# castorini/howl

Measured on AMD Instinct MI355X. Metric: utterances/sec/node (res8 end-to-end training step, 1s@16kHz, 40-mel), higher is better.
Workload: dtype f32; 1 GPU; res8 training step (frontend+fwd+xent+bwd+AdamW), 512 x 1 s utterances per GPU, 12 labels -- BASELINE configs[2] per-GPU share: res8 GSC-12, 512 x 1 s per GPU (4096 over 8); global_batch=512, samples_per_utterance=16000, labels=12, parallelism=single, frontend=eval

## Files before the change

howl_amd/csrc/res8.hip:

```cpp
#include "howl_common.hip.h"
#include "../../include/howl_hip.h"

namespace {

struct HowlPtrs6 {
    float* p[6];
};
constexpr int MAX_WINDOWS = 64;
struct HowlWinRows {
    int lo[MAX_WINDOWS], hi[MAX_WINDOWS];
};
struct HowlBnBuffers {
    float* running_mean;
    float* running_var;
    long long* num_batches;
};
struct BnFold {
    const float* part;
    int nparts;
    double count;
    float* stats_out;
    HowlBnBuffers bn;
};

// ... 1558 lines not shown
                const unsigned bc = (4u * idx[u] + 2u * h) / (unsigned)P;
                const unsigned bb = bc / NMAP;
                cc[u][h] = bc - bb * NMAP;
                if (dx == nullptr) gb[h] = dpool[bb * CP + cc[u][h]] * invP;
            }
            g[u] = dx != nullptr ? reinterpret_cast<const float4*>(dx)[idx[u]] : make_float4(gb[0], gb[0], gb[1], gb[1]);
            sv[u] = reinterpret_cast<const float4*>(s)[idx[u]];
            kk[u] = dskip != nullptr ? reinterpret_cast<const float4*>(dskip)[idx[u]] : make_float4(0.0f, 0.0f, 0.0f, 0.0f);
        }
#pragma unroll
        for (int u = 0; u < 2; ++u) {
            float2 dsa, dza, dsb, dzb;
            finish(make_float2(g[u].x, g[u].y), make_float2(sv[u].x, sv[u].y), make_float2(kk[u].x, kk[u].y), cc[u][0], dsa, dza);
            finish(make_float2(g[u].z, g[u].w), make_float2(sv[u].z, sv[u].w), make_float2(kk[u].z, kk[u].w), cc[u][1], dsb, dzb);
            if (ok[u]) {
                if (ds_out != nullptr) reinterpret_cast<float4*>(ds_out)[idx[u]] = make_float4(dsa.x, dsa.y, dsb.x, dsb.y);
                reinterpret_cast<float4*>(dz_out)[idx[u]] = make_float4(dza.x, dza.y, dzb.x, dzb.y);
            }
        }
    }
    if ((n2 & 1u) && blockIdx.x == 0 && tid == 0) {
        const unsigned i = n2 - 1;
        const unsigned bc = (2u * i) / (unsigned)P;
        const unsigned bb = bc / NMAP, c = bc - bb * NMAP;
        float2 g;
        if (dx != nullptr) {
            g = reinterpret_cast<const float2*>(dx)[i];
        } else {
            const float v = dpool[bb * CP + c] * invP;
            g = make_float2(v, v);
        }
        const float2 sv = reinterpret_cast<const float2*>(s)[i];
        const float2 kk = dskip != nullptr ? reinterpret_cast<const float2*>(dskip)[i] : make_float2(0.0f, 0.0f);
        float2 ds, dz;
        finish(g, sv, kk, c, ds, dz);
        if (ds_out != nullptr) reinterpret_cast<float2*>(ds_out)[i] = ds;
        reinterpret_cast<float2*>(dz_out)[i] = dz;
    }
}


template <bool EXACT = false>
__device__ __forceinline__ void load_feat_tile(float* tin, const float* feat, long sb, long st, long sm, int b, int T,
                                               int M, int tid, int nthreads, int t_lo = 0, int t_hi = 0) {
    const int pitch = M + 4;
    const int n = (T + 2) * pitch;
    for (int i0 = tid; i0 < n; i0 += 8 * nthreads) {
        float v[8];
#pragma unroll
        for (int j = 0; j < 8; ++j) {
            const int i = i0 + j * nthreads;
            const int t = i / pitch - 1, m = i % pitch - 1;
            const bool ok = i < n && (EXACT ? t >= t_lo && t < t_hi : t >= 0 && t < T) && m >= 0 && m < M;
            v[j] = feat[b * sb + (ok ? t * st + m * sm : 0)];
        }
#pragma unroll
        for (int j = 0; j < 8; ++j) {
            const int i = i0 + j * nthreads;
            const int t = i / pitch - 1, m = i % pitch - 1;
            const bool ok = (EXACT ? t >= t_lo && t < t_hi : t >= 0 && t < T) && m >= 0 && m < M;
            if (i < n) tin[i] = ok ? v[j] : 0.0f;
        }
    }
}

constexpr int C0M_THREADS = 512;

template <int NS = 1, bool EXACT = false>
__global__ __launch_bounds__(C0M_THREADS) void conv0_fwd_mfma_kernel(const float* __restrict__ feat, long sb, long st,
                                                                    long sm, const float* __restrict__ w0,
                                                                    float* __restrict__ s0, unsigned short* __restrict__ mask0,
                                                                    int B, int T, int M, int H, int nconv, HowlPtrs6 cw,
                                                                    float* __restrict__ wp_fwd, float* __restrict__ wp_bwd,
                                                                    int nwin, int win_step, int win_last, int slices) {
    if ((int)blockIdx.x >= nconv) {
        const int e = ((int)blockIdx.x - nconv) * C0M_THREADS + (int)threadIdx.x;
        if (e < 2 * 6 * PACK_ELEMS) pack_weights_one(cw, wp_fwd, wp_bwd, (e / PACK_ELEMS) % 6, e / (6 * PACK_ELEMS), e % PACK_ELEMS);
        return;
    }
    HIP_DYNAMIC_SHARED(float, lds)
    float* tin = lds;
    const int tid = threadIdx.x, lane = tid & 63, wave = tid >> 6;
    const int pitch = M + 4;
    const int P = H * PW;
    const int g = lane >> 4, n = lane & 15;
    float bw[3][3];
#pragma unroll
    for (int ks = 0; ks < 3; ++ks)
#pragma unroll
        for (int nt = 0; nt < 3; ++nt) {
            const int tap = 4 * ks + g, c = 16 * nt + n;
            bw[ks][nt] = (tap < 9 && c < NMAP) ? w0[c * 9 + tap] : 0.0f;
        }
    int aoff[3];
#pragma unroll
    for (int ks = 0; ks < 3; ++ks) {
        const int tap = min(4 * ks + g, 8);
        aoff[ks] = (tap / 3) * pitch + tap % 3 + (n & 7) + (n >> 3) * 3 * pitch;
    }
    for (int i = tid; i < 3 * pitch + 16; i += C0M_THREADS) tin[(T + 2) * pitch + i] = 0.0f;
    for (int item = blockIdx.x; item < B * slices; item += nconv) {
        const int b = item / slices, sl = item - b * slices;
        const int ph0 = (sl * H) / slices, ph1 = ((sl + 1) * H) / slices;
        __syncthreads();
        const int clip = b / nwin, wi = b - clip * nwin;
        const int t0 = EXACT ? wi * win_step : min(wi * win_step, win_last);
        load_feat_tile<EXACT>(tin, feat + (long)clip * sb + (long)t0 * st, 0, st, sm, 0, T, M, tid, C0M_THREADS, -t0, win_last - t0);
        __syncthreads();
        constexpr int NJ = 5 * NS;
        for (int u = wave; u < NJ * ((ph1 - ph0 + 1) / 2); u += C0M_THREADS / 64) {
            const int pp = u / NJ, j8 = u - NJ * pp;
            const float* rowp = tin + 3 * (ph0 + 2 * pp) * pitch + 8 * j8;
            {
                f32x4 acc[3][3];
#pragma unroll
                for (int tl = 0; tl < 3; ++tl)
#pragma unroll
                    for (int nt = 0; nt < 3; ++nt) acc[tl][nt] = {0.0f, 0.0f, 0.0f, 0.0f};
#pragma unroll
                for (int tl = 0; tl < 3; ++tl)
#pragma unroll
                    for (int ks = 0; ks < 3; ++ks) {
                        const float a = rowp[aoff[ks] + tl * pitch];
#pragma unroll
                        for (int nt = 0; nt < 3; ++nt)
                            acc[tl][nt] = __builtin_amdgcn_mfma_f32_16x16x4f32(a, bw[ks][nt], acc[tl][nt], 0, 0, 0);
                    }
                const int pw = 2 * j8 + (g & 1), ph = ph0 + 2 * pp + (g >> 1);
#pragma unroll
                for (int nt = 0; nt < 3; ++nt) {
                    float sum = 0.0f;
                    unsigned bits = 0;
#pragma unroll
                    for (int tl = 0; tl < 3; ++tl)
#pragma unroll
                        for (int r = 0; r < 4; ++r) {
                            const int rb = max(__float_as_int(acc[tl][nt][r]), 0);
                            sum += __int_as_float(rb);
                            bits |= min((unsigned)rb, 1u) << (4 * tl + r);
                        }
                    const int c = 16 * nt + n;
                    if (ph < ph1 && c < NMAP) {
                        const int strip = NS > 1 ? pw / PW : 0;
                        const size_t o = (((size_t)b * NS + strip) * NMAP + c) * P + (size_t)ph * PW + (pw - strip * PW);
                        s0[o] = sum * (1.0f / 12.0f);
                        if (mask0 != nullptr) mask0[o] = (unsigned short)bits;
                    }
                }
            }
        }
    }
}

constexpr int C0G_WAVES = 15, C0G_THREADS = 64 * C0G_WAVES, C0G_CPW = NMAP / C0G_WAVES;
static_assert(C0G_CPW * C0G_WAVES == NMAP, "channels split evenly over the waves");

__device__ __forceinline__ void load_patch(float (&x)[5][6], const float* tin, int pitch, int ph, int pw) {
    const float* base = tin + 3 * ph * pitch + 4 * pw;
#pragma unroll
    for (int r = 0; r < 5; ++r) {
        const float4 a = *reinterpret_cast<const float4*>(base + r * pitch);
        const float2 c = *reinterpret_cast<const float2*>(base + r * pitch + 4);
        x[r][0] = a.x, x[r][1] = a.y, x[r][2] = a.z, x[r][3] = a.w, x[r][4] = c.x, x[r][5] = c.y;
    }
}

template <int NS = 1, bool EXACT = false>
__global__ __launch_bounds__(C0G_THREADS) void conv0_wgrad_valu_kernel(const float* __restrict__ feat, long sb, long st, long sm,
                                                                      const unsigned short* __restrict__ mask0,
                                                                      const float* __restrict__ ga, const float* __restrict__ gb,
                                                                      float* __restrict__ part, int B, int T, int M, int H,
                                                                      int slices, StripGeom sg, int t_total) {
    HIP_DYNAMIC_SHARED(float, lds)
    float* tin = lds;
    const int tid = threadIdx.x, lane = tid & 63;
    const int wave = __builtin_amdgcn_readfirstlane(tid >> 6);
    const int pitch = M + 4;
    const int P = H * PW;
    float acc[C0G_CPW][9];
#pragma unroll
    for (int j = 0; j < C0G_CPW; ++j)
#pragma unroll
        for (int t = 0; t < 9; ++t) acc[j][t] = 0.0f;
    const int nrs = EXACT ? sg.nr : 1;
    for (int item = blockIdx.x; item < B * nrs * NS * slices; item += gridDim.x) {
        const int vb = item / slices, sl = item - vb * slices;
        const int vq = NS > 1 ? vb / NS : vb, strip = NS > 1 ? vb - vq * NS : 0;
        const int b = EXACT ? vq / nrs : vq, rs = EXACT ? vq - b * nrs : 0;
        const int Pv = (EXACT && rs == nrs - 1) ? sg.hv_last * PW : P;
        const int cell0 = (sl * Pv) / slices, cell1 = ((sl + 1) * Pv) / slices;
        __syncthreads();
        if constexpr (EXACT)
            load_feat_tile<true>(tin, feat + (long)rs * T * st, sb, st, sm, b, T, M, tid, C0G_THREADS, -rs * T, t_total - rs * T);
        else
            load_feat_tile(tin, feat, sb, st, sm, b, T, M, tid, C0G_THREADS);
        __syncthreads();
        const float* gab = ga + ((size_t)vb * NMAP + C0G_CPW * wave) * P;
        const float* gbb = gb != nullptr ? gb + ((size_t)vb * NMAP + C0G_CPW * wave) * P : nullptr;
        const unsigned short* mb = mask0 + ((size_t)vb * NMAP + C0G_CPW * wave) * P;
        for (int cb = cell0; cb < cell1; cb += 64) {
            const int cell = cb + lane;
            const bool valid = cell < cell1;
            const unsigned cc = (unsigned)(valid ? cell : cell1 - 1);
            float gv[C0G_CPW];
            unsigned mv[C0G_CPW];
#pragma unroll
            for (int j = 0; j < C0G_CPW; ++j) {
                const unsigned o = (unsigned)(j * P) + cc;
                gv[j] = gab[o] + (gbb != nullptr ? gbb[o] : 0.0f);
                mv[j] = mb[o];
            }
            const int ph = (int)cc / PW, pw = (int)cc - ph * PW;
            float x[5][6];
            load_patch(x, tin, pitch, ph, pw + strip * PW);
#pragma unroll
            for (int j = 0; j < C0G_CPW; ++j) {
                const int gbits = valid ? __float_as_int(gv[j] * (1.0f / 12.0f)) : 0;
#pragma unroll
                for (int tl = 0; tl < 3; ++tl)
#pragma unroll
                    for (int fl = 0; fl < 4; ++fl) {
                        const int k = 4 * tl + fl;
                        const int sel = ((int)(mv[j] << (31 - k))) >> 31;
                        const float dy = __int_as_float(sel & gbits);
#pragma unroll
                        for (int tap = 0; tap < 9; ++tap) acc[j][tap] = fmaf(dy, x[tl + tap / 3][fl + tap % 3], acc[j][tap]);
                    }
            }
        }
    }
#pragma unroll
    for (int j = 0; j < C0G_CPW; ++j)
#pragma unroll
        for (int t = 0; t < 9; ++t) {
            const float v = wave_sum_rows(acc[j][t]);
            if (lane == 0) part[(size_t)blockIdx.x * NMAP * 9 + (C0G_CPW * wave + j) * 9 + t] = v;
        }
}

constexpr int HEAD_XC = 64;
constexpr int HEAD_THREADS = 768, HEAD_PARTS = 16;
__global__ __launch_bounds__(HEAD_THREADS) void head_fwd_kernel(const float* __restrict__ s6, const float* __restrict__ stats,
                                                       const float* __restrict__ wout, const float* __restrict__ bout,
                                                       float* __restrict__ pooled, float* __restrict__ logits, int B,
                                                       int P, int C, const long long* __restrict__ labels,
                                                       float* __restrict__ nll, float* __restrict__ dlogits,
                                                       float* __restrict__ dpool, float inv_batch,
                                                       const float* __restrict__ pool, int npg, int npg_used, BnFold fold,
                                                       int ns ) {
    __shared__ float lp[CP];
    __shared__ float ll[HEAD_XC], dl[HEAD_XC], lse_s;
    __shared__ float lst[2 * CP];
    __shared__ float lw[HEAD_XC * NMAP];
    __shared__ float lparts[HEAD_PARTS][CP];
    const int tid = threadIdx.x, lane = tid & 63, wave = tid >> 6;
    const bool w_in_lds = C <= HEAD_XC;
    if (w_in_lds)
        for (int i = tid; i < C * NMAP; i += HEAD_THREADS) lw[i] = wout[i];
    if (fold.part != nullptr) {
        const int c8 = lane >> 3;
        for (int w0 = wave; w0 < CP / 4; w0 += HEAD_THREADS / 64) {
            const int c = 4 * w0 + (c8 & 3);
            const double sm = fold_part_column(fold.part, part_stride(fold.nparts), fold.nparts, (c8 < 4 ? 0 : CP) + c, lane);
            const double q = __shfl_xor(sm, 32);
            if (c8 < 4 && (lane & 7) == 0) {
                const double mean = sm / fold.count;
                double var = q / fold.count - mean * mean;
                var = var < 0.0 ? 0.0 : var;
                const float fm = (c < NMAP) ? (float)mean : 0.0f;
                const float fr = (c < NMAP) ? (float)(1.0 / sqrt(var + (double)BN_EPS)) : 0.0f;
                lst[c] = fm;
                lst[CP + c] = fr;
                if (blockIdx.x == 0) {
                    fold.stats_out[c] = fm;
                    fold.stats_out[CP + c] = fr;
                    if (c < NMAP && fold.bn.running_mean != nullptr) {
                        const double unbiased = fold.count > 1.0 ? var * fold.count / (fold.count - 1.0) : var;
                        fold.bn.running_mean[c] = (1.0f - BN_MOMENTUM) * fold.bn.running_mean[c] + BN_MOMENTUM * (float)mean;
                        fold.bn.running_var[c] = (1.0f - BN_MOMENTUM) * fold.bn.running_var[c] + BN_MOMENTUM * (float)unbiased;
                    }
                    if (c == 0 && fold.bn.num_batches != nullptr) fold.bn.num_batches[0] += 1;
                }
            }
        }
    } else if (tid < 2 * CP) {
        lst[tid] = stats[tid];
    }
    __syncthreads();
    for (int b = blockIdx.x; b < B; b += gridDim.x) {
        __syncthreads();
        if (pool != nullptr) {
            const int nparts = ns * npg_used;
            const int pc = tid % CP, pk = tid / CP;
            float acc = 0.0f;
            for (int k0 = 0; k0 < nparts; k0 += HEAD_PARTS) {
                const int k = k0 + pk;
                if (k < nparts) {
                    const int sgi = k / npg_used, g = k - sgi * npg_used;
                    lparts[pk][pc] = pool[(((size_t)b * ns + sgi) * npg + g) * CP + pc];
                }
                __syncthreads();
                if (tid < CP) {
                    const int n = nparts - k0 < HEAD_PARTS ? nparts - k0 : HEAD_PARTS;
                    for (int j = 0; j < n; ++j) acc += lparts[j][tid];
                }
                __syncthreads();
            }
            if (tid < CP) {
                const float v = tid < NMAP ? (acc / (float)P - lst[tid]) * lst[CP + tid] : 0.0f;
                lp[tid] = v;
                pooled[(size_t)b * CP + tid] = v;
            }
        } else if (wave < 4)
        for (int c0 = wave; c0 < CP; c0 += 12) {
            float a8[3][8];
#pragma unroll
            for (int u = 0; u < 3; ++u) {
                const int c = c0 + 4 * u < NMAP ? c0 + 4 * u : NMAP - 1;
                const float* src = s6 + ((size_t)b * NMAP + c) * P;
#pragma unroll
                for (int j = 0; j < 8; ++j) a8[u][j] = src[min(lane + 64 * j, P - 1)];
            }
#pragma unroll
            for (int u = 0; u < 3; ++u) {
                const int c = c0 + 4 * u;
#pragma unroll
                for (int j = 0; j < 8; ++j) a8[u][j] = (lane + 64 * j < P) ? fabsf(a8[u][j]) : 0.0f;
                float acc = ((a8[u][0] + a8[u][1]) + (a8[u][2] + a8[u][3])) + ((a8[u][4] + a8[u][5]) + (a8[u][6] + a8[u][7]));
                acc = wave_sum(acc);
                const float v = c < NMAP ? (acc / (float)P - lst[c]) * lst[CP + c] : 0.0f;
                if (lane == 0 && c < CP) {
                    lp[c] = v;
                    pooled[(size_t)b * CP + c] = v;
                }
            }
        }
        __syncthreads();
        for (int k = tid; k < C; k += HEAD_THREADS) {
            float acc = bout[k];
            if (w_in_lds)
                for (int c = 0; c < NMAP; ++c) acc = fmaf(lw[k * NMAP + c], lp[c], acc);
            else
                for (int c = 0; c < NMAP; ++c) acc = fmaf(wout[k * NMAP + c], lp[c], acc);
            logits[(size_t)b * C + k] = acc;
            if (labels != nullptr) ll[k] = acc;
        }
        if (labels == nullptr) continue;
        __syncthreads();
        const int y = (int)labels[b];
        if (tid == 0) {
            float mx = ll[0];
            for (int k = 1; k < C; ++k) mx = fmaxf(mx, ll[k]);
            float se = 0.0f;
            for (int k = 0; k < C; ++k) se += expf(ll[k] - mx);
            const float lse = mx + logf(se);
            lse_s = lse;
            nll[b] = lse - ll[y];
        }
        __syncthreads();
        if (tid < C) {
            const float d = (expf(ll[tid] - lse_s) - (tid == y ? 1.0f : 0.0f)) * inv_batch;
            dl[tid] = d;
            dlogits[(size_t)b * C + tid] = d;
        }
        __syncthreads();
        if (tid < CP) {
            float acc = 0.0f;
            if (tid < NMAP)
                for (int k = 0; k < C; ++k) acc = fmaf(dl[k], lw[k * NMAP + tid], acc);
            dpool[(size_t)b * CP + tid] = acc;
        }
    }
}

__global__ __launch_bounds__(256) void head_fwd_windows_kernel(const float* __restrict__ s6, const float* __restrict__ stats,
                                                               const float* __restrict__ wout, const float* __restrict__ bout,
                                                               float* __restrict__ logits, int B, int nwin, int Hw,
                                                               HowlWinRows rows, float inv_count, int C, int ns) {
    __shared__ float lp[CP];
    const int tid = threadIdx.x, lane = tid & 63, wave = tid >> 6;
    const int Pw = Hw * PW;
    for (int b = blockIdx.x; b < B; b += gridDim.x) {
        __syncthreads();
        for (int c = wave; c < CP; c += 4) {
            float acc = 0.0f;
            if (c < NMAP) {
                for (int w = 0; w < nwin * ns; ++w) {
                    const float* src = s6 + ((size_t)(b * nwin * ns + w) * NMAP + c) * Pw;
                    for (int i = rows.lo[w / ns] * PW + lane; i < rows.hi[w / ns] * PW; i += 64) acc += fabsf(src[i]);
                }
// ... 142 lines not shown
    if ((threadIdx.x & 63) == 0) red[threadIdx.x >> 6] = acc;
    __syncthreads();
    if (threadIdx.x == 0) {
        double tot = 0.0;
        for (int w = 0; w < 16; ++w) tot += red[w];
        loss[0] = (float)(tot / (double)B);
    }
}

__global__ void adamw_kernel(float* __restrict__ p, const float* __restrict__ g, float* __restrict__ m,
                             float* __restrict__ v, size_t n, HowlAdamWCoef c) {
    for (size_t i = (size_t)blockIdx.x * blockDim.x + threadIdx.x; i < n; i += (size_t)gridDim.x * blockDim.x)
        howl_adamw_element(p, m, v, i, g[i], c);
}

}

namespace {

size_t conv0_tile_floats(int T, int M) { return (size_t)(T + 2) * (M + 4) + 3 * (M + 4) + 16; }
size_t conv_lds_bytes(int H, bool own_rows) {
    return (size_t)(3 * KSTEPS * 64 + tile_floats(H, own_rows) + 4 * CP + 12 * 2 * 16) * sizeof(float);
}
size_t wgrad_lds_bytes(int H) { return (size_t)(tile_floats_z(H) + tile_floats_x(H) + 6 * CP) * sizeof(float); }

struct Ws {
    float* wp_fwd;
    float* wp_bwd;
    float* part;
    float* part2;
    float* stats;
    float* m12;
    float* dpool;
    float* pool;
    float* bufa;
    float* bufb;
    float* dz;
    float* dz2;
    float* dsa;
    float* dsb;
    float* wpart;
    float* c0part;
};

size_t ws_layout(Ws* w, char* base, int B, int H, int G, int cus, size_t* fwd_eval_bytes) {
    size_t off = 0;
    auto take = [&](size_t floats) {
        float* p = base ? reinterpret_cast<float*>(base + off) : nullptr;
        off += ((floats * sizeof(float) + 255) / 256) * 256;
        return p;
    };
    const size_t act = (size_t)B * NMAP * H * PW;
    w->wp_fwd = take((size_t)6 * 3 * KSTEPS * 64);
    w->wp_bwd = take((size_t)6 * 3 * KSTEPS * 64);
    const int max_parts = G > cus ? G : cus;
    w->part = take((size_t)part_stride(max_parts) * 2 * CP);
    w->part2 = take((size_t)part_stride(max_parts) * 2 * CP);
    w->stats = take((size_t)6 * 2 * CP);
    w->m12 = take(2 * CP);
    w->dpool = take((size_t)B * CP);
    w->pool = take((size_t)B * 16 * CP);
    *fwd_eval_bytes = off;
    w->bufa = take(act);
    w->bufb = take(act);
    w->dz = take(act);
    w->dz2 = take(act);
    w->dsa = take(act);
    w->dsb = take(act);
    w->wpart = take((size_t)6 * G * CP * WNCOL);
    w->c0part = take((size_t)max_parts * NMAP * 9);
    return off;
}

int mel_strips(int M) { return M == 40 ? 1 : (M == 80 ? 2 : 0); }
int even_grid(int g, int strips) { return strips > 1 ? ((g & ~1) > 2 ? (g & ~1) : 2) : g; }
int launch_blocks(int nblk, int per_group) { return 8 * per_group * ((nblk + 7) / 8); }
int conv_slices(int nblk, int H, int budget) {
    const int ntiles = (H * PW + 15) / 16;
    for (int sl = 4; sl > 1; sl >>= 1)
        if (nblk * sl <= budget && 4 * sl <= ntiles) return sl;
    return 1;
}
void pair_slices(int nblk, int H, int cus, int* sd, int* sw) {
    const int ntiles = (H * PW + 15) / 16;
    const int opts[3][2] = {{4, 2}, {2, 2}, {2, 1}};
    *sd = *sw = 1;
    for (const auto& o : opts)
        if (nblk * (o[0] + o[1]) <= cus && 4 * o[0] <= ntiles) {
            *sd = o[0];
            *sw = o[1];
            return;
        }
}
int conv0_slices(int B, int cus) {
    const int sl = cus / (B > 0 ? B : 1);
    return sl < 1 ? 1 : (sl > 8 ? 8 : sl);
}
bool env_off(const char* name) {
    const char* e = getenv(name);
    return e != nullptr && e[0] == '0';
}

constexpr int WIN_H = MAX_H, WIN_MARGIN = 7, WIN_STEP = WIN_H - 2 * WIN_MARGIN;
int long_windows(int H) { return H <= WIN_H ? 1 : (H - WIN_H + WIN_STEP - 1) / WIN_STEP + 1; }

struct Res8Plan {
    int B, T, M, ns, nr, Hs, hv_last, Bv, halo;
    StripGeom sg;
    int P, Pt;
    bool slicing, merged, fused;
    int G, SL;
    size_t lds_conv;
    int Bw, Tw, S0, G0, c0_nwin, c0_step, c0_last;
    bool c0_exact;
    size_t lds_conv0;
    int Gh, SD, SW, ew_grid;
    bool fold_in_pair;
    size_t wpart_stride, lds_wgrad, lds_pair;
    int S0w, G0w;
    size_t lds_conv0w;
    size_t saved_floats, train_bytes, eval_bytes;
    size_t long_map_bytes, long_bytes;
    Ws ws;
};

void plan_launches(Res8Plan& p, bool slice_conv0, char* ws_base) {
    const int cus = howl_num_cus(), H = p.Hs;
    p.P = H * PW;
    p.Pt = (p.T / 3) * PW * p.ns;
    p.saved_floats = (size_t)p.Bv * NMAP * p.P;
    p.slicing = !env_off("HOWL_RES8_SLICES");
    p.merged = !env_off("HOWL_RES8_BWD_PAIR");
    p.fused = p.halo != 0 || !env_off("HOWL_RES8_BWD_FUSED");

    p.G = even_grid(p.Bv < cus ? p.Bv : cus, p.ns);
    p.SL = p.halo == 0 && p.slicing ? conv_slices(p.G, H, cus) : 1;
    p.lds_conv = conv_lds_bytes(H, p.halo == 2);
    p.S0 = slice_conv0 && p.slicing ? conv0_slices(p.Bw, cus) : 1;
    p.G0 = p.Bw * p.S0 < 2 * cus ? p.Bw * p.S0 : 2 * cus;
    p.lds_conv0 = conv0_tile_floats(p.Tw, p.M) * sizeof(float);

    const int half = cus / 2 > 0 ? cus / 2 : 1;
    p.Gh = even_grid(p.Bv < half ? p.Bv : half, p.ns);
    p.SD = p.SW = 1;
    if (p.halo == 0 && p.slicing) pair_slices(p.Gh, H, cus, &p.SD, &p.SW);
    p.fold_in_pair = p.Gh * p.SD >= 64;
    p.wpart_stride = (size_t)p.Gh * CP * WNCOL;
    p.lds_wgrad = wgrad_lds_bytes(H);
    p.lds_pair = p.lds_conv > p.lds_wgrad ? p.lds_conv : p.lds_wgrad;
    const size_t quads = (p.saved_floats / 4 + BRB_THREADS - 1) / BRB_THREADS;
    p.ew_grid = quads < 1 ? 1 : (quads > (size_t)(2 * cus) ? 2 * cus : (int)quads);
    p.S0w = p.slicing ? conv0_slices(p.Bv, cus) : 1;
    p.G0w = p.Bv * p.S0w < cus ? p.Bv * p.S0w : cus;
    p.lds_conv0w = ((size_t)(p.Tw + 2) * (p.M + 4) + 16) * sizeof(float);

    p.train_bytes = ws_layout(&p.ws, ws_base, p.Bv, H, p.G, cus, &p.eval_bytes);
}

Res8Plan res8_plan(int B, int T, int M, void* ws = nullptr) {
    Res8Plan p{};
    const int H = T / 3;
    p.B = B, p.T = T, p.M = M;
    p.ns = mel_strips(M) > 0 ? mel_strips(M) : 1;
    p.nr = H <= MAX_H ? 1 : (H + MAX_H - 1) / MAX_H;
    p.Hs = (H + p.nr - 1) / p.nr;
    p.hv_last = H - (p.nr - 1) * p.Hs;
    p.Bv = B * p.nr * p.ns;
    p.halo = p.nr > 1 ? 2 : (p.ns > 1 ? 1 : 0);
    p.sg = StripGeom{p.nr, p.ns, p.hv_last};
    p.c0_exact = p.halo == 2;
    p.Bw = B * p.nr;
    p.Tw = p.c0_exact ? 3 * p.Hs : T;
    p.c0_nwin = p.c0_exact ? p.nr : 1;
    p.c0_step = p.c0_exact ? 3 * p.Hs : 0;
    p.c0_last = p.c0_exact ? T : 0;
    plan_launches(p, true, static_cast<char*>(ws));
    return p;
}

Res8Plan res8_long_plan(int B, int T, int M, void* ws = nullptr) {
    Res8Plan p{};
    const int H = T / 3, nw = long_windows(H);
    p.B = B, p.T = T, p.M = M;
    p.ns = mel_strips(M) > 0 ? mel_strips(M) : 1;
    p.nr = 1, p.Hs = p.hv_last = WIN_H;
    p.Bv = B * nw * p.ns;
    p.halo = p.ns > 1 ? 1 : 0;
    p.sg = StripGeom{1, 1, 0};
    p.Bw = B * nw;
    p.Tw = 3 * WIN_H + T % 3;
    p.c0_nwin = nw, p.c0_step = 3 * WIN_STEP, p.c0_last = 3 * (H - WIN_H);
    static_assert((6 * 2 * CP * sizeof(float)) % 256 == 0, "statistics block keeps the 256-byte alignment");
    p.long_map_bytes = ((size_t)p.Bv * NMAP * WIN_H * PW * sizeof(float) + 255) / 256 * 256;
    const size_t front = 3 * p.long_map_bytes + 6 * 2 * CP * sizeof(float) + 256;
    plan_launches(p, false, ws ? static_cast<char*>(ws) + front : nullptr);
    p.long_bytes = front + p.train_bytes;
    return p;
}

int check_workspace(const char* who, size_t have, size_t need) {
    if (have >= need) return HOWL_OK;
    howl_set_error("%s: workspace %zu < %zu bytes", who, have, need);
    return HOWL_E_WORKSPACE;
}
template <class T>
HowlPtrs6 ptrs6(T* const (&a)[6]) {
    HowlPtrs6 r;
    for (int i = 0; i < 6; ++i) r.p[i] = const_cast<float*>(a[i]);
    return r;
}
StageCfg plain_tile(const float* t) { return StageCfg{t, nullptr, nullptr, nullptr, nullptr, 0.0f, false, false, false}; }

template <auto Kernel>
void raise_lds_limit(size_t lds) {
    static thread_local size_t granted[16] = {};
    howl_raise_lds(reinterpret_cast<const void*>(Kernel), lds, granted, "res8 kernel");
}
template <int HALO>
StripGeom geom_arg(const Res8Plan& p) { return HALO == 2 ? p.sg : StripGeom{1, 1, 0}; }

struct Conv3x3Launch {
    StageCfg in;
    const float* in_stats = nullptr;
    const float* wp = nullptr;
    const float* res = nullptr;
    float* out = nullptr;
    const float* xs = nullptr;
    const float* xs_stats = nullptr;
    float* part = nullptr;
    float* pool = nullptr;
    BnFold fold{};
    BwdFold bfold{};
    WFold wf{nullptr, 0, nullptr};
};
template <int MODE, int SLICES, int HALO>
void launch_conv3x3_inst(const Res8Plan& p, hipStream_t stream, const Conv3x3Launch& a) {
    const int nblk = MODE == 0 ? p.G : p.Gh;
    raise_lds_limit<conv3x3_mfma_kernel<MODE, SLICES, HALO>>(p.lds_conv);
    hipLaunchKernelGGL((conv3x3_mfma_kernel<MODE, SLICES, HALO>), dim3(launch_blocks(nblk, SLICES)), dim3(CONV_THREADS), p.lds_conv,
                       stream, a.in, a.in_stats, a.wp, a.res, a.out, a.xs, a.xs_stats, a.part, a.pool, p.Bv, p.Hs, nblk, a.fold,
                       a.bfold, a.wf, geom_arg<HALO>(p));
}
template <int MODE>
void launch_conv3x3(const Res8Plan& p, hipStream_t stream, const Conv3x3Launch& a) {
    const int slices = MODE == 0 ? p.SL : p.SD;
    if (p.halo == 2)
        launch_conv3x3_inst<MODE, 1, 2>(p, stream, a);
    else if (p.halo == 1)
        launch_conv3x3_inst<MODE, 1, 1>(p, stream, a);
    else if (slices == 4)
        launch_conv3x3_inst<MODE, 4, 0>(p, stream, a);
    else if (slices == 2)
        launch_conv3x3_inst<MODE, 2, 0>(p, stream, a);
    else
        launch_conv3x3_inst<MODE, 1, 0>(p, stream, a);
}

struct BwdLayerLaunch {
    StageCfg zc;
    BwdFold bfold;
    const float* wp;
    float* dx;
    const float* xs;
    const float* xs_stats;
    float* spart;
    const float* s_prev;
    const float* in_stats;
    float* wpart;
    WFold wf;
};
template <int SD, int SW, int HALO>
void launch_pair_inst(const Res8Plan& p, hipStream_t stream, const BwdLayerLaunch& a) {
    raise_lds_limit<bwd_pair_kernel<SD, SW, HALO>>(p.lds_pair);
    hipLaunchKernelGGL((bwd_pair_kernel<SD, SW, HALO>), dim3(launch_blocks(p.Gh, SD + SW)), dim3(CONV_THREADS), p.lds_pair, stream, a.zc,
                       a.bfold, a.wp, a.dx, a.xs, a.xs_stats, a.spart, a.s_prev, a.in_stats, a.wpart, p.Bv, p.Hs, p.Gh, a.wf,
                       geom_arg<HALO>(p));
}
void launch_pair(const Res8Plan& p, hipStream_t stream, const BwdLayerLaunch& a) {
    if (p.halo == 2)
        launch_pair_inst<1, 1, 2>(p, stream, a);
    else if (p.halo == 1)
        launch_pair_inst<1, 1, 1>(p, stream, a);
    else if (p.SD == 4 && p.SW == 2)
        launch_pair_inst<4, 2, 0>(p, stream, a);
    else if (p.SD == 2 && p.SW == 2)
        launch_pair_inst<2, 2, 0>(p, stream, a);
    else if (p.SD == 2 && p.SW == 1)
        launch_pair_inst<2, 1, 0>(p, stream, a);
    else
        launch_pair_inst<1, 1, 0>(p, stream, a);
}
template <int SW, int HALO>
void launch_wgrad_inst(const Res8Plan& p, hipStream_t stream, const BwdLayerLaunch& a) {
    StageCfg zw = a.zc;
    zw.ds = nullptr;
    raise_lds_limit<wgrad_mfma_kernel<SW, HALO>>(p.lds_wgrad);
    hipLaunchKernelGGL((wgrad_mfma_kernel<SW, HALO>), dim3(launch_blocks(p.Gh, SW)), dim3(CONV_THREADS), p.lds_wgrad, stream,
                       WStage{zw, a.s_prev, false}, a.in_stats, a.bfold, a.wpart, p.Bv, p.Hs, p.Gh, geom_arg<HALO>(p));
}
void launch_wgrad(const Res8Plan& p, hipStream_t stream, const BwdLayerLaunch& a) {
    if (p.halo == 2)
        launch_wgrad_inst<1, 2>(p, stream, a);
    else if (p.halo == 1)
        launch_wgrad_inst<1, 1>(p, stream, a);
    else if (p.SW == 2)
        launch_wgrad_inst<2, 0>(p, stream, a);
    else
        launch_wgrad_inst<1, 0>(p, stream, a);
}

struct Feat {
    const float* x;
    long sb, st, sm;
};
template <int NS, bool EXACT>
void launch_conv0_fwd_inst(const Res8Plan& p, hipStream_t stream, const Feat& f, const HowlRes8Params* prm, float* s0,
                           unsigned short* mask0) {
    const int npack = (2 * 6 * PACK_ELEMS + C0M_THREADS - 1) / C0M_THREADS;
    hipLaunchKernelGGL((conv0_fwd_mfma_kernel<NS, EXACT>), dim3(p.G0 + npack), dim3(C0M_THREADS), p.lds_conv0, stream, f.x, f.sb, f.st,
                       f.sm, prm->conv0_w, s0, mask0, p.Bw, p.Tw, p.M, p.Hs, p.G0, ptrs6(prm->conv_w), p.ws.wp_fwd, p.ws.wp_bwd,
                       p.c0_nwin, p.c0_step, p.c0_last, p.S0);
}
void launch_conv0_fwd(const Res8Plan& p, hipStream_t stream, const Feat& f, const HowlRes8Params* prm, float* s0,
                      unsigned short* mask0) {
    if (p.c0_exact && p.ns == 2)
        launch_conv0_fwd_inst<2, true>(p, stream, f, prm, s0, mask0);
    else if (p.c0_exact)
        launch_conv0_fwd_inst<1, true>(p, stream, f, prm, s0, mask0);
    else if (p.ns == 2)
        launch_conv0_fwd_inst<2, false>(p, stream, f, prm, s0, mask0);
    else
        launch_conv0_fwd_inst<1, false>(p, stream, f, prm, s0, mask0);
}
template <int NS, bool EXACT>
void launch_conv0_wgrad_inst(const Res8Plan& p, hipStream_t stream, const Feat& f, const unsigned short* mask0, const float* g0) {
    hipLaunchKernelGGL((conv0_wgrad_valu_kernel<NS, EXACT>), dim3(p.G0w), dim3(C0G_THREADS), p.lds_conv0w, stream, f.x, f.sb, f.st, f.sm,
                       mask0, g0, (const float*)nullptr, p.ws.c0part, p.B, p.Tw, p.M, p.Hs, p.S0w, p.sg, p.T);
}
void launch_conv0_wgrad(const Res8Plan& p, hipStream_t stream, const Feat& f, const unsigned short* mask0, const float* g0) {
    if (p.c0_exact && p.ns == 2)
        launch_conv0_wgrad_inst<2, true>(p, stream, f, mask0, g0);
    else if (p.c0_exact)
        launch_conv0_wgrad_inst<1, true>(p, stream, f, mask0, g0);
    else if (p.ns == 2)
        launch_conv0_wgrad_inst<2, false>(p, stream, f, mask0, g0);
    else
        launch_conv0_wgrad_inst<1, false>(p, stream, f, mask0, g0);
}

int res8_fwd_impl(const HowlRes8Params* prm, const Feat& feat, int B, int T, int M, int C, int training, const HowlRes8Saved* sv,
                  float* logits, void* ws, size_t ws_bytes, const long long* labels, float* nll, float* dlogits, hipStream_t stream) {
    HOWL_REQUIRE(prm && feat.x && sv && logits && ws, "howl_res8_fwd: null pointer");
    HOWL_REQUIRE(labels == nullptr || (nll != nullptr && dlogits != nullptr && C <= HEAD_XC),
                 "howl_res8_fwd_xent: nll / dlogits missing or more than %d classes (C=%d)", HEAD_XC, C);
    HOWL_REQUIRE(mel_strips(M) > 0, "howl_res8_fwd: res8 pools (3,4) over 40 or 80 mel bins; got M=%d", M);
    HOWL_REQUIRE(B >= 1 && T / 3 >= 1, "howl_res8_fwd: B=%d T=%d unsupported (T >= 3)", B, T);
    HOWL_REQUIRE(C >= 1, "howl_res8_fwd: C must be positive");
    const Res8Plan p = res8_plan(B, T, M, ws);
    HOWL_REQUIRE(p.hv_last >= 1 && p.nr <= MAX_ROW_STRIPS, "howl_res8_fwd: T=%d frames unsupported (%d row strips)", T, p.nr);
    if (int rc = check_workspace("howl_res8_fwd", ws_bytes, training ? p.train_bytes : p.eval_bytes)) return rc;
    const Ws& w = p.ws;
    if (!training)
        hipLaunchKernelGGL(bn_eval_stats_kernel, dim3(6), dim3(64), 0, stream, ptrs6(prm->bn_running_mean), ptrs6(prm->bn_running_var),
                           sv->bn_stats);
    {
        HowlProfScope prof("conv0_fwd", stream);
        launch_conv0_fwd(p, stream, feat, prm, sv->s[0], sv->mask0);
    }
    const double count = (double)B * (double)p.Pt;
    const auto fold_of = [&](int layer, float* part) {
        return BnFold{part, p.G * p.SL, count, sv->bn_stats + (size_t)(layer - 1) * 2 * CP,
                      HowlBnBuffers{prm->bn_running_mean[layer - 1], prm->bn_running_var[layer - 1], prm->bn_num_batches[layer - 1]}};
    };
    for (int i = 1; i <= 6; ++i) {
        Conv3x3Launch a;
        a.in = plain_tile(sv->s[i - 1]);
        a.wp = w.wp_fwd + (size_t)(i - 1) * 3 * KSTEPS * 64;
        a.res = (i % 2) == 0 ? sv->s[i - 2] : nullptr;
        a.out = sv->s[i];
        a.part = training ? ((i & 1) ? w.part : w.part2) : nullptr;
        a.pool = i == 6 ? w.pool : nullptr;
        if (i > 1 && training)
            a.fold = fold_of(i - 1, (i & 1) ? w.part2 : w.part);
        else if (i > 1)
            a.in_stats = sv->bn_stats + (size_t)(i - 2) * 2 * CP;
        HowlProfScope prof("conv3x3_fwd", stream);
        launch_conv3x3<0>(p, stream, a);
    }
    const int groups = 4 * p.SL;
    hipLaunchKernelGGL(head_fwd_kernel, dim3(B < 1024 ? B : 1024), dim3(HEAD_THREADS), 0, stream, sv->s[6],
                       sv->bn_stats + (size_t)5 * 2 * CP, prm->out_w, prm->out_b, sv->pooled, logits, B, p.Pt, C, labels, nll, dlogits,
                       w.dpool, 1.0f / (float)B, (const float*)w.pool, groups, groups < (p.P + 15) / 16 ? groups : (p.P + 15) / 16,
                       training ? fold_of(6, w.part2) : BnFold{}, p.nr * p.ns);
    HOWL_CHECK_LAUNCH("howl_res8_fwd");
    return HOWL_OK;
}

int res8_bwd_impl(const HowlRes8Params* prm, const Feat& feat, int B, int T, int M, int C, const HowlRes8Saved* sv, const float* dlogits,
                  const HowlRes8Grads* gr, void* ws, size_t ws_bytes, int part, const float* nll, float* loss, hipStream_t stream,
                  const HowlAdamW* adamw = nullptr) {
    HOWL_REQUIRE(prm && feat.x && sv && dlogits && gr && ws, "howl_res8_bwd: null pointer");
    HOWL_REQUIRE(adamw == nullptr || (part == 0 && adamw->p && adamw->g && adamw->m && adamw->v && adamw->n >= 1 && adamw->step >= 1),
                 "howl_res8_bwd: HowlAdamW needs the whole pass (part 0) and complete buffers");
    HOWL_REQUIRE(part >= 0 && part <= 2, "howl_res8_bwd_part: part must be 0 (all), 1 or 2");
    const bool run_layers = part != 2, run_conv0 = part != 1;
    HOWL_REQUIRE(mel_strips(M) > 0, "howl_res8_bwd: M must be 40 or 80 (got %d)", M);
    HOWL_REQUIRE(B >= 1 && T / 3 >= 1, "howl_res8_bwd: B=%d T=%d unsupported", B, T);
    const Res8Plan p = res8_plan(B, T, M, ws);
    HOWL_REQUIRE(p.hv_last >= 1 && p.nr <= MAX_ROW_STRIPS, "howl_res8_bwd: T=%d frames unsupported (%d row strips)", T, p.nr);
    if (int rc = check_workspace("howl_res8_bwd", ws_bytes, p.train_bytes)) return rc;
    HOWL_REQUIRE(p.saved_floats / 2 < (size_t)1 << 31, "howl_res8_bwd: B=%d too large for the 32-bit element index of the elementwise pass", B);
    const Ws& w = p.ws;
    const double count = (double)B * (double)p.Pt;

    if (run_layers) {
        if (nll == nullptr)
            hipLaunchKernelGGL(head_bwd_pool_kernel, dim3((B * CP + 255) / 256), dim3(256), 0, stream, dlogits, prm->out_w, w.dpool,
                               B, C);
        hipLaunchKernelGGL(head_bwd_param_kernel, dim3(C + (nll != nullptr ? 2 : 1)), dim3(1024), 0, stream, dlogits, sv->pooled,
                           w.dpool, gr->out_w, gr->out_b, w.m12, B, C, p.Pt, nll, loss);
    }
    float* dx_cur = nullptr;
    float* dx_next = w.bufa;
    float* ds_prev = nullptr;
    float* ds_free = w.dsa;
    for (int i = 6; i >= 1; --i) {
        const bool even = (i % 2) == 0;
        const float* stats_i = sv->bn_stats + (size_t)(i - 1) * 2 * CP;
        float* ds_out = even ? ds_free : nullptr;
        float* dz = even ? w.dz : w.dz2;
        float* part_in = p.fused ? ((i & 1) ? w.part2 : w.part) : w.part;
        float* part_out = p.fused ? ((i & 1) ? w.part : w.part2) : w.part;
        BwdLayerLaunch a;
        a.bfold = BwdFold{stats_i, w.m12, i == 6 ? (const float*)nullptr : (const float*)part_in, p.Gh * p.SD, count};
        a.zc = plain_tile(dz);
        if (p.fused)
            a.zc = StageCfg{dx_cur, sv->s[i], even ? (const float*)ds_prev : (const float*)nullptr, ds_out, w.dpool,
                            1.0f / (float)p.Pt, true, even, false};
        else if (run_layers)
            hipLaunchKernelGGL(bn_relu_bwd_kernel, dim3(p.ew_grid), dim3(BRB_THREADS), 0, stream, (const float*)dx_cur, w.dpool, sv->s[i],
                               stats_i, w.m12, a.bfold.part, p.Gh * p.SD, count, even ? (const float*)ds_prev : (const float*)nullptr,
                               even ? 1 : 0, ds_out, dz, B, p.P);
        if (even) {
            float* t = ds_prev ? ds_prev : w.dsb;
            ds_prev = ds_out;
            ds_free = t;
        }
        const bool need_stats = i > 1;
        a.s_prev = sv->s[i - 1];
        a.in_stats = need_stats ? sv->bn_stats + (size_t)(i - 2) * 2 * CP : nullptr;
        a.wp = w.wp_bwd + (size_t)(i - 1) * 3 * KSTEPS * 64;
        a.dx = dx_next;
        a.xs = need_stats ? sv->s[i - 1] : (const float*)ds_prev;
        a.xs_stats = a.in_stats;
        a.spart = need_stats ? part_out : nullptr;
        a.wpart = w.wpart + (size_t)(i - 1) * p.wpart_stride;
        a.wf = (p.fold_in_pair && i < 6) ? WFold{w.wpart + (size_t)i * p.wpart_stride, p.Gh, gr->conv_w[i]} : WFold{nullptr, 0, nullptr};
        if (!run_layers) {
        } else if (p.merged) {
            HowlProfScope prof("bwd_pair", stream);
            launch_pair(p, stream, a);
        } else {
            {
                HowlProfScope prof("conv3x3_dgrad", stream);
                Conv3x3Launch d;
                d.in = a.zc, d.wp = a.wp, d.out = a.dx, d.xs = a.xs, d.xs_stats = a.xs_stats, d.part = a.spart;
                d.bfold = a.bfold, d.wf = a.wf;
                launch_conv3x3<1>(p, stream, d);
            }
            HowlProfScope prof("wgrad", stream);
            launch_wgrad(p, stream, a);
        }
        dx_cur = dx_next;
        dx_next = (dx_next == w.bufa) ? w.bufb : w.bufa;
    }
    HOWL_REQUIRE(sv->mask0 != nullptr, "howl_res8_bwd: saved->mask0 is required");
    const HowlPtrs6 gw = ptrs6(gr->conv_w);
    const RowsAdamW no_opt{nullptr, nullptr, nullptr, nullptr, HowlAdamWCoef{}, 0, 0, 0};
    const auto reduce_rows = [&](int cols, int first, int skip, int nrows, const RowsAdamW& opt) {
        hipLaunchKernelGGL(reduce_rows_all_kernel, dim3((cols + 63) / 64, nrows + (opt.on ? 1 : 0)), dim3(1024), 0, stream,
                           (const float*)w.wpart, p.wpart_stride, p.Gh, gw, (const float*)w.c0part, p.G0w, gr->conv0_w, first, skip,
                           nrows, opt);
    };
    if (part == 1)
        reduce_rows(CP * WNCOL, 0, 0, p.fold_in_pair ? 1 : 6, no_opt);
    if (run_conv0) {
        {
            HowlProfScope prof("conv0_wgrad", stream);
            launch_conv0_wgrad(p, stream, feat, sv->mask0, dx_cur);
        }
// ... 146 lines not shown
```

Baseline: 472,100 utterances/sec.

## Rewrite conv0 weight-gradient kernel on MFMA with double-buffered feature tiles

Measured after the change: 474,600 utterances/sec (median of 6 runs). Within noise of the previous version (+0.5%).

```diff
diff --git a/howl_amd/csrc/res8.hip b/howl_amd/csrc/res8.hip
--- a/howl_amd/csrc/res8.hip
+++ b/howl_amd/csrc/res8.hip
@@ -1734,90 +1734,174 @@
     }
 }
 
-constexpr int C0G_WAVES = 15, C0G_THREADS = 64 * C0G_WAVES, C0G_CPW = NMAP / C0G_WAVES;
-static_assert(C0G_CPW * C0G_WAVES == NMAP, "channels split evenly over the waves");
-
-__device__ __forceinline__ void load_patch(float (&x)[5][6], const float* tin, int pitch, int ph, int pw) {
-    const float* base = tin + 3 * ph * pitch + 4 * pw;
-#pragma unroll
-    for (int r = 0; r < 5; ++r) {
-        const float4 a = *reinterpret_cast<const float4*>(base + r * pitch);
-        const float2 c = *reinterpret_cast<const float2*>(base + r * pitch + 4);
-        x[r][0] = a.x, x[r][1] = a.y, x[r][2] = a.z, x[r][3] = a.w, x[r][4] = c.x, x[r][5] = c.y;
-    }
-}
+constexpr int C0W_WAVES = 12, C0W_THREADS = 64 * C0W_WAVES;
+constexpr int c0w_tile_regs(int ns) { return ((3 * MAX_H + 4) * (40 * ns + 4) + C0W_THREADS - 1) / C0W_THREADS; }
+int c0w_table_cells(int H) { return 16 * ((H * PW + 15) / 16); }
+size_t c0w_tile_floats(int T, int M) {
+    const size_t tiles = 2 * (size_t)(T + 2) * (M + 4), comb = (size_t)C0W_THREADS * 4;
+    return tiles > comb ? tiles : comb;
+}
+size_t conv0_wgrad_lds_bytes(int T, int M) { return (c0w_tile_floats(T, M) + c0w_table_cells(T / 3)) * sizeof(float); }
+
+template <bool EXACT, int PITCH, int NR>
+__device__ __forceinline__ void fetch_feat_tile(float (&v)[NR], unsigned& okbits, const float* feat, long sb, long st, long sm, int b,
+                                                int T, int tid, int nthreads, int t_lo, int t_hi) {
+    constexpr int pitch = PITCH, M = PITCH - 4;
+    const int n = (T + 2) * pitch;
+    okbits = 0;
+#pragma unroll
+    for (int j = 0; j < NR; ++j) {
+        const int i = tid + j * nthreads;
+        const int t = i / pitch - 1, m = i % pitch - 1;
+        const bool ok = i < n && (EXACT ? t >= t_lo && t < t_hi : t >= 0 && t < T) && m >= 0 && m < M;
+        v[j] = feat[b * sb + (ok ? t * st + m * sm : 0)];
+        okbits |= (ok ? 1u : 0u) << j;
+    }
+}
+template <int NR>
+__device__ __forceinline__ void store_feat_tile(float* tin, const float (&v)[NR], unsigned okbits, int n, int tid, int nthreads) {
+#pragma unroll
+    for (int j = 0; j < NR; ++j) {
+        const int i = tid + j * nthreads;
+        if (i < n) tin[i] = ((okbits >> j) & 1u) ? v[j] : 0.0f;
+    }
+}
+
+struct C0wOps {
+    float2 g[2];
+    unsigned m[2];
+};
 
 template <int NS = 1, bool EXACT = false>
-__global__ __launch_bounds__(C0G_THREADS) void conv0_wgrad_valu_kernel(const float* __restrict__ feat, long sb, long st, long sm,
+__global__ __launch_bounds__(C0W_THREADS) void conv0_wgrad_mfma_kernel(const float* __restrict__ feat, long sb, long st, long sm,
                                                                       const unsigned short* __restrict__ mask0,
-                                                                      const float* __restrict__ ga, const float* __restrict__ gb,
-                                                                      float* __restrict__ part, int B, int T, int M, int H,
-                                                                      int slices, StripGeom sg, int t_total) {
+                                                                      const float* __restrict__ g0, float* __restrict__ part, int B,
+                                                                      int T, int M, int H, int slices, StripGeom sg, int t_total) {
     HIP_DYNAMIC_SHARED(float, lds)
-    float* tin = lds;
+    constexpr int PITCH = 40 * NS + 4, NR = c0w_tile_regs(NS);
     const int tid = threadIdx.x, lane = tid & 63;
     const int wave = __builtin_amdgcn_readfirstlane(tid >> 6);
-    const int pitch = M + 4;
+    const int n = lane & 15, g = lane >> 4;
+    const int nt = wave % 3, ql = wave / 3;
     const int P = H * PW;
-    float acc[C0G_CPW][9];
-#pragma unroll
-    for (int j = 0; j < C0G_CPW; ++j)
-#pragma unroll
-        for (int t = 0; t < 9; ++t) acc[j][t] = 0.0f;
+    const int tile = (T + 2) * PITCH;
+    const int c = min(16 * nt + n, NMAP - 1);
+    const int tap = min(n, 8);
+    const int btap = (tap / 3) * PITCH + tap % 3;
+    f32x4 acc = {0.0f, 0.0f, 0.0f, 0.0f};
+    const int ntab = 16 * ((P + 15) / 16);
+    const size_t tile2 = 2 * (size_t)tile, comb = (size_t)C0W_THREADS * 4;
+    int* const tab = reinterpret_cast<int*>(lds + (tile2 > comb ? tile2 : comb));
+    for (int i = tid; i < ntab; i += C0W_THREADS) {
+        const int cc = min(i, P - 1), ph = cc / PW;
+        tab[i] = 4 * (3 * ph * PITCH + 4 * (cc - ph * PW));
+    }
     const int nrs = EXACT ? sg.nr : 1;
-    for (int item = blockIdx.x; item < B * nrs * NS * slices; item += gridDim.x) {
+    const int nitems = B * nrs * NS * slices;
+    float tv[NR];
+    unsigned tok = 0;
+    auto fetch_tile = [&](int item) {
+        const int vq = (item / slices) / NS;
+        const int b = EXACT ? vq / nrs : vq, rs = EXACT ? vq - b * nrs : 0;
+        if constexpr (EXACT)
+            fetch_feat_tile<true, PITCH>(tv, tok, feat + (long)rs * T * st, sb, st, sm, b, T, tid, C0W_THREADS, -rs * T, t_total - rs * T);
+        else
+            fetch_feat_tile<false, PITCH>(tv, tok, feat, sb, st, sm, b, T, tid, C0W_THREADS, 0, 0);
+    };
+    int cell0 = 0, cell1 = 0, Q1 = 0, q = 0, strip = 0, rot = 0;
+    const float* grow = g0;
+    const unsigned short* mrow = mask0;
+    C0wOps cur = {}, nxt = {};
+    auto load_ops = [&](int qq) {
+        C0wOps o;
+#pragma unroll
+        for (int h = 0; h < 2; ++h) {
+            const int hc = 16 * qq + 4 * g + 2 * h;
+            const int off = hc + 2 <= P ? hc : 0;
+            o.g[h] = *reinterpret_cast<const float2*>(grow + off);
+            o.m[h] = *reinterpret_cast<const unsigned*>(mrow + off);
+        }
+        return o;
+    };
+    auto begin_item = [&](int item) {
         const int vb = item / slices, sl = item - vb * slices;
-        const int vq = NS > 1 ? vb / NS : vb, strip = NS > 1 ? vb - vq * NS : 0;
-        const int b = EXACT ? vq / nrs : vq, rs = EXACT ? vq - b * nrs : 0;
+        const int vq = NS > 1 ? vb / NS : vb;
+        strip = NS > 1 ? vb - vq * NS : 0;
+        const int rs = EXACT ? vq % nrs : 0;
         const int Pv = (EXACT && rs == nrs - 1) ? sg.hv_last * PW : P;
-        const int cell0 = (sl * Pv) / slices, cell1 = ((sl + 1) * Pv) / slices;
+        cell0 = (sl * Pv) / slices, cell1 = ((sl + 1) * Pv) / slices;
+        const int Q0 = cell0 >> 4;
+        Q1 = (cell1 + 15) >> 4;
+        grow = g0 + ((size_t)vb * NMAP + c) * P;
+        mrow = mask0 + ((size_t)vb * NMAP + c) * P;
+        q = Q0 + ((ql - rot) & 3);
+        rot = (rot + Q1 - Q0) & 3;
+        if (q < Q1) cur = load_ops(q);
+    };
+    if ((int)blockIdx.x < nitems) {
+        begin_item(blockIdx.x);
+        fetch_tile(blockIdx.x);
+        store_feat_tile(lds, tv, tok, tile, tid, C0W_THREADS);
+    }
+    int it = 0;
+    for (int item = blockIdx.x; item < nitems; item += gridDim.x, ++it) {
+        const char* tin = reinterpret_cast<const char*>(lds + (it & 1) * tile) + 4 * (btap + 4 * strip * PW);
         __syncthreads();
-        if constexpr (EXACT)
-            load_feat_tile<true>(tin, feat + (long)rs * T * st, sb, st, sm, b, T, M, tid, C0G_THREADS, -rs * T, t_total - rs * T);
-        else
-            load_feat_tile(tin, feat, sb, st, sm, b, T, M, tid, C0G_THREADS);
-        __syncthreads();
-        const float* gab = ga + ((size_t)vb * NMAP + C0G_CPW * wave) * P;
-        const float* gbb = gb != nullptr ? gb + ((size_t)vb * NMAP + C0G_CPW * wave) * P : nullptr;
-        const unsigned short* mb = mask0 + ((size_t)vb * NMAP + C0G_CPW * wave) * P;
-        for (int cb = cell0; cb < cell1; cb += 64) {
-            const int cell = cb + lane;
-            const bool valid = cell < cell1;
-            const unsigned cc = (unsigned)(valid ? cell : cell1 - 1);
-            float gv[C0G_CPW];
-            unsigned mv[C0G_CPW];
-#pragma unroll
-            for (int j = 0; j < C0G_CPW; ++j) {
-                const unsigned o = (unsigned)(j * P) + cc;
-                gv[j] = gab[o] + (gbb != nullptr ? gbb[o] : 0.0f);
-                mv[j] = mb[o];
+        const int next = item + gridDim.x;
+        if (next < nitems) fetch_tile(next);
+        for (; q < Q1; q += 4) {
+            HOWL_OPAQUE_V(cur.g[0].x);
+            HOWL_OPAQUE_V(cur.g[0].y);
+            HOWL_OPAQUE_V(cur.g[1].x);
+            HOWL_OPAQUE_V(cur.g[1].y);
+            HOWL_OPAQUE_V(cur.m[0]);
+            HOWL_OPAQUE_V(cur.m[1]);
+            HOWL_SCHED_PIN();
+            if (q + 4 < Q1) nxt = load_ops(q + 4);
+            int boff[4];
+#pragma unroll
+            for (int j = 0; j < 4; ++j) boff[j] = tab[16 * q + 4 * g + j];
+            if (16 * q < cell0 || 16 * q + 16 > cell1) {
+#pragma unroll
+                for (int j = 0; j < 4; ++j) {
+                    const int cell = 16 * q + 4 * g + j;
+                    if (cell < cell0 || cell >= cell1) cur.m[j >> 1] &= (j & 1) ? 0x0000ffffu : 0xffff0000u;
+                }
             }
-            const int ph = (int)cc / PW, pw = (int)cc - ph * PW;
-            float x[5][6];
-            load_patch(x, tin, pitch, ph, pw + strip * PW);
-#pragma unroll
-            for (int j = 0; j < C0G_CPW; ++j) {
-                const int gbits = valid ? __float_as_int(gv[j] * (1.0f / 12.0f)) : 0;
+            int gbits[4];
+#pragma unroll
+            for (int j = 0; j < 4; ++j) gbits[j] = __float_as_int(((j & 1) ? cur.g[j >> 1].y : cur.g[j >> 1].x) * (1.0f / 12.0f));
+#pragma unroll
+            for (int j = 0; j < 4; ++j)
 #pragma unroll
                 for (int tl = 0; tl < 3; ++tl)
 #pragma unroll
                     for (int fl = 0; fl < 4; ++fl) {
-                        const int k = 4 * tl + fl;
-                        const int sel = ((int)(mv[j] << (31 - k))) >> 31;
-                        const float dy = __int_as_float(sel & gbits);
-#pragma unroll
-                        for (int tap = 0; tap < 9; ++tap) acc[j][tap] = fmaf(dy, x[tl + tap / 3][fl + tap % 3], acc[j][tap]);
+                        const int bit = 16 * (j & 1) + 4 * tl + fl;
+                        const int sel = ((int)(cur.m[j >> 1] << (31 - bit))) >> 31;
+                        const float a = __int_as_float(sel & gbits[j]);
+                        const float x = *reinterpret_cast<const float*>(tin + boff[j] + 4 * (tl * PITCH + fl));
+                        acc = __builtin_amdgcn_mfma_f32_16x16x4f32(a, x, acc, 0, 0, 0);
                     }
-            }
-        }
-    }
-#pragma unroll
-    for (int j = 0; j < C0G_CPW; ++j)
-#pragma unroll
-        for (int t = 0; t < 9; ++t) {
-            const float v = wave_sum_rows(acc[j][t]);
-            if (lane == 0) part[(size_t)blockIdx.x * NMAP * 9 + (C0G_CPW * wave + j) * 9 + t] = v;
-        }
+            cur = nxt;
+        }
+        if (next < nitems) {
+            begin_item(next);
+            store_feat_tile(lds + ((it + 1) & 1) * tile, tv, tok, tile, tid, C0W_THREADS);
+        }
+    }
+    __syncthreads();
+#pragma unroll
+    for (int r = 0; r < 4; ++r) lds[(wave * 4 + r) * 64 + lane] = acc[r];
+    __syncthreads();
+    if (tid < NMAP * 9) {
+        const int co = tid / 9, tp = tid - 9 * co;
+        const int row = co & 15, src = (row >> 2) * 16 + tp;
+        float s = 0.0f;
+#pragma unroll
+        for (int i = 0; i < 4; ++i) s += lds[(((co >> 4) + 3 * i) * 4 + (row & 3)) * 64 + src];
+        part[(size_t)blockIdx.x * NMAP * 9 + tid] = s;
+    }
 }
 
 constexpr int HEAD_XC = 64;
@@ -2266,7 +2350,7 @@
     p.ew_grid = quads < 1 ? 1 : (quads > (size_t)(2 * cus) ? 2 * cus : (int)quads);
     p.S0w = p.slicing ? conv0_slices(p.Bv, cus) : 1;
     p.G0w = p.Bv * p.S0w < cus ? p.Bv * p.S0w : cus;
-    p.lds_conv0w = ((size_t)(p.Tw + 2) * (p.M + 4) + 16) * sizeof(float);
+    p.lds_conv0w = conv0_wgrad_lds_bytes(p.Tw, p.M);
 
     p.train_bytes = ws_layout(&p.ws, ws_base, p.Bv, H, p.G, cus, &p.eval_bytes);
 }
@@ -2448,8 +2532,8 @@
 }
 template <int NS, bool EXACT>
 void launch_conv0_wgrad_inst(const Res8Plan& p, hipStream_t stream, const Feat& f, const unsigned short* mask0, const float* g0) {
-    hipLaunchKernelGGL((conv0_wgrad_valu_kernel<NS, EXACT>), dim3(p.G0w), dim3(C0G_THREADS), p.lds_conv0w, stream, f.x, f.sb, f.st, f.sm,
-                       mask0, g0, (const float*)nullptr, p.ws.c0part, p.B, p.Tw, p.M, p.Hs, p.S0w, p.sg, p.T);
+    hipLaunchKernelGGL((conv0_wgrad_mfma_kernel<NS, EXACT>), dim3(p.G0w), dim3(C0W_THREADS), p.lds_conv0w, stream, f.x, f.sb, f.st, f.sm,
+                       mask0, g0, p.ws.c0part, p.B, p.Tw, p.M, p.Hs, p.S0w, p.sg, p.T);
 }
 void launch_conv0_wgrad(const Res8Plan& p, hipStream_t stream, const Feat& f, const unsigned short* mask0, const float* g0) {
     if (p.c0_exact && p.ns == 2)
```
